# plurigrid/moose

Measured on AMD Instinct MI355X. Metric: replicated fixed(14,23) matmul elems/sec, higher is better.
Workload: dtype fixed(14,23) over Z_2^128 (exact multi-modular int8-MFMA GEMM)

## Files before the change

csrc/gemm_crt.hip:

```cpp
#include <hip/hip_runtime.h>

#include <algorithm>
#include <cmath>
#include <cstdint>
#include <cstdlib>
#include <cstring>
#include <mutex>

#include "hip_attr.h"
#include "moosex.h"
#include "prf_dev.h"
#include "rss_fused.h"

void mx_ws_note(int dev, int64_t want, bool ok);
bool mx_ws_malloc(void** p, int64_t bytes);
void mx_ws_shared_note(void);

namespace {

using u64 = uint64_t;
using u128 = unsigned __int128;
typedef int v4i __attribute__((ext_vector_type(4)));
typedef int v16i __attribute__((ext_vector_type(16)));

// ... 262 lines not shown
    const int r = (int)((g >> 2) & (ROWS - 1));
    const int64_t q = g / (ROWS * 4);
    const int64_t kb = q % nkb, t = q / nkb;
    const int64_t row = t * ROWS + r;
    const int64_t k0 = kb * BK + c * 16;
    uint32_t v[16][NW];
#pragma unroll
    for (int j = 0; j < 16; ++j) {
      const int64_t k = k0 + j;
      T e = 0;
      if (row < R) {
        if (!TRANS) {
          if (k < K) e = mode == 2 ? (T)(x0[row * K + k] + x1[row * K + k]) : x0[row * K + k];
          else if (mode == 1 && k < 2 * K) e = x1[row * K + (k - K)];
        } else {
          if (k < K)
            e = (mode & 1) ? (T)(x0[k * R + row] + x1[k * R + row]) : x0[k * R + row];
          else if (mode == 1 && k < 2 * K) e = x0[(k - K) * R + row];
          else if (mode == 2 && k < 2 * K) e = x1[(k - K) * R + row];
        }
      }
#pragma unroll
      for (int w = 0; w < NW; ++w) v[j][w] = (uint32_t)(e >> (32 * w));
    }
    const int64_t boff = (t * nkb_s + kb) * (int64_t)(ROWS * BK) + img_off(r, c);
    auto emit = [&](int8_t* base) __attribute__((always_inline)) {
    {
      int rr[16];
#pragma unroll
      for (int j = 0; j < 16; ++j) rr[j] = (int)(v[j][0] * tab.mul0);
      v4i o;
#pragma unroll
      for (int u = 0; u < 4; ++u) o[u] = (int)pack4(rr[4 * u], rr[4 * u + 1], rr[4 * u + 2], rr[4 * u + 3]);
      *(v4i*)base = o;
    }
    for (int i = 1; i < n; ++i) {
      const uint32_t w[4] = {tab.w[i][0], tab.w[i][1], tab.w[i][2], tab.w[i][3]};
      const uint32_t neg = tab.neg[i];
      const float p = (float)tab.p[i], rcp = tab.rcp[i];
      int rr[16];
      if constexpr (PK) {
#pragma unroll
        for (int j = 0; j < 16; j += 2)
          residue2<NW>(v[j], v[j + 1], w, neg, p, rcp, rr[j], rr[j + 1]);
      } else {
#pragma unroll
        for (int j = 0; j < 16; ++j) rr[j] = residue<NW>(v[j], w, neg, p, rcp);
      }
      v4i o;
#pragma unroll
      for (int u = 0; u < 4; ++u) o[u] = (int)pack4(rr[4 * u], rr[4 * u + 1], rr[4 * u + 2], rr[4 * u + 3]);
      *(v4i*)(base + i * plane) = o;
    }
    };
    emit(ob + boff);
    if (src.n > 0 && src.dual[b]) {
#pragma unroll
      for (int j = 0; j < 16; ++j) {
        const int64_t k = k0 + j;
        if (row < R && k < K) {
          T e = 0;
#pragma unroll
          for (int w = 0; w < NW; ++w) e |= (T)v[j][w] << (32 * w);
          e += TRANS ? x1[k * R + row] : x1[row * K + k];
#pragma unroll
          for (int w = 0; w < NW; ++w) v[j][w] = (uint32_t)(e >> (32 * w));
        }
      }
      emit(ob + src.dual[b] + boff);
    }
  }
}

struct ShareSrc {
  const void* x = nullptr;
  int kind = 0;
  int frac = 0;
  int j0 = 0;
  uint64_t nonce = 0;
  mxd::KeySrc key;
};
struct SrcPlan {
  const void* x;
  int kind, pad;
  double scale;
  uint64_t nonce;
  int ph[4];
  int64_t off[4];
};

template <bool TRANS, int ROWS, bool PK>
__global__ void __launch_bounds__(256)
    k_crt_prep_src(const SrcPlan s, const mxd::KeySrc keys, int64_t R, int64_t K,
                   int8_t* __restrict__ out, int64_t tiles, int64_t nkb, const PrepTab tab) {
  using T = u128;
  constexpr int NW = 4;
  __shared__ uint32_t rks[1][mxd::kKeyWords];
  __shared__ uint4 xch[4][4][64];
  mxd::stage_keys(rks, keys, 1);
  const int lane = threadIdx.x & 63;
  const int p = lane & 3;
  uint4(*xw)[64] = xch[threadIdx.x >> 6];
  const int n = tab.n;
  const int64_t plane = tiles * nkb * (int64_t)(ROWS * BK);
  const int64_t total = tiles * ROWS * nkb * 4;
  for (int64_t g = blockIdx.x * (int64_t)blockDim.x + threadIdx.x; g < total;
       g += (int64_t)gridDim.x * blockDim.x) {
    const int c = (int)((g >> 2) & 3);
    const int rlow = (int)((g >> 4) & 3);
    const int64_t rest = g >> 6;
    int64_t row, kb, i0, istep;
    if (!TRANS) {
      const int64_t q = rest / (ROWS / 4);
      kb = 4 * (q % (nkb / 4)) + p;
      row = (q / (nkb / 4)) * ROWS + (rest % (ROWS / 4)) * 4 + rlow;
      i0 = row * K + (kb - p) * BK + c * 16;
      istep = 1;
    } else {
      const int64_t q = rest >> 4;
      kb = q % nkb;
      row = (q / nkb) * 256 + 64 * p + (rest & 15) * 4 + rlow;
      i0 = (kb * BK + c * 16) * R + (row - 64 * p);
      istep = R;
    }
    const bool live = row < R;
    const int64_t t = row / ROWS;
    const int r = (int)(row % ROWS);
    uint32_t rr[16][NW], v[16][NW];
#pragma unroll
    for (int jj = 0; jj < 4; ++jj) {
      uint32_t w[16];
      mx::chacha_block(rks[0], s.nonce, mx::ks_block_of((uint64_t)(i0 + (4 * jj + p) * istep)), w);
#pragma unroll
      for (int q = 0; q < 4; ++q)
        xw[q][lane ^ q] = make_uint4(w[4 * q], w[4 * q + 1], w[4 * q + 2], w[4 * q + 3]);
      __builtin_amdgcn_fence(__ATOMIC_RELEASE, "wavefront");
      __builtin_amdgcn_wave_barrier();
      __builtin_amdgcn_fence(__ATOMIC_ACQUIRE, "wavefront");
#pragma unroll
      for (int u = 0; u < 4; ++u) {
        const uint4 e = xw[p][((lane & ~3) | u) ^ p];
        rr[4 * jj + u][0] = live ? e.x : 0u;
        rr[4 * jj + u][1] = live ? e.y : 0u;
        rr[4 * jj + u][2] = live ? e.z : 0u;
        rr[4 * jj + u][3] = live ? e.w : 0u;
      }
      __builtin_amdgcn_fence(__ATOMIC_RELEASE, "wavefront");
      __builtin_amdgcn_wave_barrier();
      __builtin_amdgcn_fence(__ATOMIC_ACQUIRE, "wavefront");
    }
    float kf[16];
    T xp[16];
    if (s.kind == MX_SHARE_F64) {
      double d[16];
#pragma unroll
      for (int j = 0; j < 16; ++j)
        d[j] = live ? ((const double*)s.x)[i0 + 64 * p + j * istep] : 0.0;
#pragma unroll
      for (int j = 0; j < 16; ++j) xp[j] = mxf::share_plain<T>(MX_SHARE_F64, d, j, s.scale);
    } else {
#pragma unroll
      for (int j = 0; j < 16; ++j)
        xp[j] = live ? mxf::share_plain<T>(s.kind, s.x, i0 + 64 * p + j * istep, s.scale) : (T)0;
    }
#pragma unroll
    for (int j = 0; j < 16; ++j) {
      T h = 0;
#pragma unroll
      for (int w = 0; w < NW; ++w) h |= (T)rr[j][w] << (32 * w);
      const T x = xp[j];
      const T other = mxf::share_masked<T>(s.kind, x, h);
#pragma unroll
      for (int w = 0; w < NW; ++w) v[j][w] = (uint32_t)(other >> (32 * w));
      kf[j] = (float)crt_sum_kappa(rr[j][NW - 1], v[j][NW - 1],
                                   (uint32_t)((T)(h + other) >> (32 * (NW - 1))));
    }
    const int64_t boff = (t * nkb + kb) * (int64_t)(ROWS * BK) + img_off(r, c);
    bool has[4];
#pragma unroll
    for (int ph = 0; ph < 4; ++ph)
      has[ph] = s.ph[0] == ph || s.ph[1] == ph || s.ph[2] == ph || s.ph[3] == ph;
    const bool do_r = has[0] || has[2], do_v = has[1] || has[2];
    auto put = [&](int ph, int64_t ioff, const v4i o) __attribute__((always_inline)) {
#pragma unroll
      for (int e = 0; e < 4; ++e)
        if (s.ph[e] == ph) *(v4i*)(out + s.off[e] + ioff + boff) = o;
    };
    auto pack16 = [](const int (&q)[16]) __attribute__((always_inline)) {
      v4i o;
#pragma unroll
      for (int u = 0; u < 4; ++u) o[u] = (int)pack4(q[4 * u], q[4 * u + 1], q[4 * u + 2], q[4 * u + 3]);
      return o;
    };
    const v4i zero = {0, 0, 0, 0};
    {
      int q[16];
#pragma unroll
      for (int j = 0; j < 16; ++j) q[j] = (int)(rr[j][0] * tab.mul0);
      put(0, 0, pack16(q));
#pragma unroll
      for (int j = 0; j < 16; ++j) q[j] = (int)(v[j][0] * tab.mul0);
      put(1, 0, pack16(q));
#pragma unroll
      for (int j = 0; j < 16; ++j) q[j] = (int)((rr[j][0] + v[j][0]) * tab.mul0);
      put(2, 0, pack16(q));
      put(3, 0, zero);
    }
    for (int i = 1; i < n; ++i) {
      const uint32_t w[4] = {tab.w[i][0], tab.w[i][1], tab.w[i][2], tab.w[i][3]};
      const uint32_t neg = tab.neg[i];
      const float pf = (float)tab.p[i], rcp = tab.rcp[i];
      const int64_t ioff = i * plane;
      const float nf = (float)neg;
      auto res4 = [&](const uint32_t (&x)[16][NW], int u, float (&f)[4])
                      __attribute__((always_inline)) {
        if constexpr (PK) {
#pragma unroll
          for (int j = 0; j < 4; j += 2) {
            const f2 g = residue2_f<NW>(x[4 * u + j], x[4 * u + j + 1], w, neg, pf, rcp);
            f[j] = g.x;
            f[j + 1] = g.y;
          }
        } else {
#pragma unroll
          for (int j = 0; j < 4; ++j) f[j] = residue_f<NW>(x[4 * u + j], w, neg, pf, rcp);
        }
      };
      v4i o_r, o_v, o_s;
#pragma unroll
      for (int u = 0; u < 4; ++u) {
        float fr[4], fv[4], fs[4];
        if (do_r) {
          res4(rr, u, fr);
          o_r[u] = (int)pack4((int)fr[0], (int)fr[1], (int)fr[2], (int)fr[3]);
        }
        if (do_v) {
          res4(v, u, fv);
          o_v[u] = (int)pack4((int)fv[0], (int)fv[1], (int)fv[2], (int)fv[3]);
        }
        if (has[2]) {
          if constexpr (PK) {
#pragma unroll
            for (int j = 0; j < 4; j += 2) {
              const f2 g = crt_combine2((f2){fr[j], fr[j + 1]}, (f2){fv[j], fv[j + 1]},
                                        (f2){kf[4 * u + j], kf[4 * u + j + 1]}, nf, pf, rcp);
              fs[j] = g.x;
              fs[j + 1] = g.y;
            }
          } else {
#pragma unroll
            for (int j = 0; j < 4; ++j)
              fs[j] = crt_combine_f(fr[j], fv[j], kf[4 * u + j], nf, pf, rcp);
          }
          o_s[u] = (int)pack4((int)fs[0], (int)fs[1], (int)fs[2], (int)fs[3]);
        }
      }
      put(0, ioff, o_r);
      put(1, ioff, o_v);
      put(2, ioff, o_s);
      put(3, ioff, zero);
    }
  }
}

template <class T>
__global__ void __launch_bounds__(256)
    k_add_pair(const T* __restrict__ a, const T* __restrict__ b, T* __restrict__ o, int64_t n) {
  for (int64_t i = blockIdx.x * (int64_t)blockDim.x + threadIdx.x; i < n;
       i += (int64_t)gridDim.x * blockDim.x)
    o[i] = a[i] + b[i];
}

__device__ inline int64_t xcd_remap(int64_t bid, int64_t nwg) {
  const int64_t q = nwg / 8, r = nwg % 8;
  const int64_t x = bid % 8;
  return (x < r ? x * (q + 1) : r * (q + 1) + (x - r) * q) + bid / 8;
}

constexpr int waitcnt_vm_lgkm0(int vm) { return (vm & 15) | ((vm >> 4) << 14) | (7 << 4); }

__device__ __forceinline__ int centered_mod(int acc, float pf, float rcp, int t16) {
  const int hi = acc >> 16, lo = acc & 0xffff;
  const int s = __mul24(hi, t16) + lo;
  const float fs = (float)s;
  const float qt = __builtin_rintf(fs * rcp);
  return (int)__builtin_fmaf(-qt, pf, fs);
}

template <int WR, int WC, int BN, int MINW>
// ... 158 lines not shown
      qs[e] = 0.f;
#pragma unroll
      for (int k = 0; k < NK; ++k) acc[e][k] = 0;
    }
    const int8_t* src = CR + b * n * ntiles * (int64_t)kCrTile + off;
    for (int i = 0; i < n; ++i) {
      const uint2 v = *(const uint2*)(src + i * ntiles * (int64_t)kCrTile);
      const float rcp = rc.rcp[i];
      int wk[NK];
#pragma unroll
      for (int k = 0; k < NK; ++k) wk[k] = rc.W[i][k];
#pragma unroll
      for (int e = 0; e < 8; ++e) {
        const int c = (int)(int8_t)(((e < 4 ? v.x : v.y) >> (8 * (e & 3))) & 0xff);
        qs[e] = __builtin_fmaf((float)c, rcp, qs[e]);
#pragma unroll
        for (int k = 0; k < NK; ++k) acc[e][k] += __mul24(c, wk[k]);
      }
    }
    const int64_t tm = tile / tiles_n, tn = tile % tiles_n;
    const int bi = blk / NBJ, bj = blk % NBJ;
    const int64_t gcol = tn * BN + bj * 32 + (lane & 31);
    T mw = 0;
#pragma unroll
    for (int k = 0; k < NK; ++k) mw |= (T)rc.Mw[k] << (16 * k);
#pragma unroll
    for (int e = 0; e < 8; ++e) {
      const int ee = hf * 8 + e;
      const int row = (ee & 3) + 8 * (ee >> 2) + 4 * (lane >> 5);
      const int64_t grow = tm * BM + bi * 32 + row;
      T z = 0;
#pragma unroll
      for (int k = 0; k < NK; ++k) z += (T)(int64_t)acc[e][k] << (16 * k);
      const int q = (int)__builtin_rintf(qs[e]);
      z -= (T)(int64_t)q * mw;
      if (grow < M && gcol < N) {
        T* pc = C + (b * M + grow) * N + gcol;
        *pc = accumulate ? (T)(*pc + z) : z;
      }
    }
  }
}

template <int WR, int WC, int BN, int MINW, int STG = kStages, int IL = 0>
__global__ void __launch_bounds__(64 * WR * WC, MINW)
    k_crt_gemm16(const int8_t* __restrict__ RA, const int8_t* __restrict__ RB,
                 int8_t* __restrict__ CR, int tiles_m, int tiles_n, int nkb_all, int gM,
                 const EpiTab ep, int dma_mask, int bcast, int a_nkb, int roll, int amap,
                 int bmap) {
  constexpr int NW = WR * WC;
  constexpr int MI = BM / WR / 16, NJ = BN / WC / 16;
  constexpr int NM = MI * NJ;
  constexpr int kImgB = BN * BK;
  constexpr int kStageBytes = kImg + kImgB;
  constexpr int NPIECE = kStageBytes / 1024;
  constexpr int PPW = NPIECE / NW;
  static_assert(PPW * NW == NPIECE, "stage pieces must split evenly over the waves");
  extern __shared__ __attribute__((aligned(16))) int8_t smem[];
  const int ntiles = tiles_m * tiles_n;
  const int tid_flat = (int)xcd_remap(blockIdx.x, ntiles);
  const int group = tid_flat / (gM * tiles_n);
  const int first_m = group * gM;
  const int gm = tiles_m - first_m < gM ? tiles_m - first_m : gM;
  const int in_group = tid_flat % (gM * tiles_n);
  const int tm = first_m + in_group % gm, tn = in_group / gm;
  const int g = amap < 0 ? (int)((blockIdx.y + ep.n) % gridDim.y) : (int)blockIdx.y;
  const int mi = g % ep.n;
  int nkb = nkb_all;
  const int8_t* ga = RA + ((int64_t)((bcast & 1) ? mi : g) * tiles_m + tm) * a_nkb * (int64_t)kImg;
  const int8_t* gb = RB + ((int64_t)((bcast & 2) ? mi : g) * tiles_n + tn) * nkb_all * (int64_t)kImgB;
  const int8_t* ga2 = ga;
  const int8_t* gb2 = gb;
  int khalf = 1 << 30;
  if (roll) {
    const int nbt = (int)gridDim.y / ep.n;
    const int b2 = (g / ep.n + roll) % nbt;
    ga2 = RA + ((int64_t)(b2 * ep.n + mi) * tiles_m + tm) * a_nkb * (int64_t)kImg -
          (int64_t)a_nkb * kImg;
    khalf = a_nkb;
  } else if (amap < 0) {
    const int sh = 8 * (g / ep.n);
    const int e1 = (amap >> sh) & 7, e2 = (amap >> (sh + 3)) & 7;
    const int f1 = (bmap >> sh) & 7, f2 = (bmap >> (sh + 3)) & 7;
    ga = RA + ((int64_t)(e1 * ep.n + mi) * tiles_m + tm) * a_nkb * (int64_t)kImg;
    ga2 = RA + ((int64_t)(e2 * ep.n + mi) * tiles_m + tm) * a_nkb * (int64_t)kImg -
          (int64_t)a_nkb * kImg;
    gb = RB + ((int64_t)(f1 * ep.n + mi) * tiles_n + tn) * a_nkb * (int64_t)kImgB;
    gb2 = RB + ((int64_t)(f2 * ep.n + mi) * tiles_n + tn) * a_nkb * (int64_t)kImgB -
          (int64_t)a_nkb * kImgB;
    khalf = a_nkb;
    if ((amap >> (sh + 6)) & 1) nkb = a_nkb;
  }

  const int lane = threadIdx.x & 63;
  const int wave = __builtin_amdgcn_readfirstlane(threadIdx.x >> 6);
  const int wr = wave / WC, wc = wave % WC;
  const int co = 16 * ((lane >> 4) ^ swz((lane & 15) >> 2));
  const int rowa = (wr * (BM / WR) + (lane & 15)) * BK + co;
  const int rowb = kImg + (wc * (BN / WC) + (lane & 15)) * BK + co;

  const int8_t* srcs[PPW];
  const int8_t* srcs2[PPW];
  int dsts[PPW], steps[PPW];
#pragma unroll
  for (int t = 0; t < PPW; ++t) {
    const int pc = wave + NW * t;
    const bool is_b = pc >= 16;
    const int pp = is_b ? pc - 16 : pc;
    srcs[t] = (is_b ? gb : ga) + pp * 1024 + lane * 16;
    srcs2[t] = (is_b ? gb2 : ga2) + pp * 1024 + lane * 16;
    dsts[t] = (is_b ? kImg : 0) + pp * 1024;
    steps[t] = is_b ? kImgB : kImg;
  }
  bool dma_on[PPW];
#pragma unroll
  for (int t = 0; t < PPW; ++t) dma_on[t] = (dma_mask >> ((wave + NW * t) >= 16 ? 1 : 0)) & 1;
  auto dma = [&](int kb, int t, int8_t* dst_stage) {
    if (!dma_on[t]) return;
    const int8_t* src = kb >= khalf ? srcs2[t] : srcs[t];
    __builtin_amdgcn_global_load_lds((const void*)(src + (int64_t)kb * steps[t]),
                                     (__attribute__((address_space(3))) void*)(dst_stage + dsts[t]),
                                     16, 0, 0);
  };

  v4i acc[MI][NJ];
#pragma unroll
  for (int i = 0; i < MI; ++i)
#pragma unroll
    for (int j = 0; j < NJ; ++j) acc[i][j] = v4i{0, 0, 0, 0};

  v4i fa0[MI], fb0[NJ], fa1[MI], fb1[NJ];
  const bool no_frags = (dma_mask & 8) != 0;
  auto frags = [&](const int8_t* st, v4i(&fa)[MI], v4i(&fb)[NJ]) {
    if (no_frags) return;
#pragma unroll
    for (int i = 0; i < MI; ++i) fa[i] = *(const v4i*)(st + rowa + i * 16 * BK);
#pragma unroll
    for (int j = 0; j < NJ; ++j) fb[j] = *(const v4i*)(st + rowb + j * 16 * BK);
  };

  constexpr int PRO = IL == 3 ? 4 : STG;
#pragma unroll
  for (int s = 0; s < PRO; ++s)
#pragma unroll
    for (int t = 0; t < PPW; ++t) dma(s < nkb ? s : nkb - 1, t, smem + s * kStageBytes);
  __builtin_amdgcn_s_waitcnt(waitcnt_vm_lgkm0((PRO - 1) * PPW));
  __builtin_amdgcn_s_barrier();
  __builtin_amdgcn_sched_barrier(0);
  frags(smem, fa0, fb0);

  auto step = [&](int kb, int8_t* cur, int8_t* nxt, v4i(&fa)[MI], v4i(&fb)[NJ], v4i(&na)[MI],
                  v4i(&nbf)[NJ]) __attribute__((always_inline)) {
    const int kn = kb + STG < nkb ? kb + STG : nkb - 1;
#pragma unroll MI
    for (int i = 0; i < MI; ++i) {
      if (i == MI / 2) {
        __builtin_amdgcn_s_waitcnt(waitcnt_vm_lgkm0((STG - 2) * PPW));
        __builtin_amdgcn_s_barrier();
        __builtin_amdgcn_sched_barrier(0);
        frags(nxt, na, nbf);
        __builtin_amdgcn_sched_barrier(0);
      }
#pragma unroll NJ
      for (int j = 0; j < NJ; ++j) {
        acc[i][j] = __builtin_amdgcn_mfma_i32_16x16x64_i8(fa[i], fb[j], acc[i][j], 0, 0, 0);
        __builtin_amdgcn_sched_barrier(0);
        const int h = (i - MI / 2) * NJ + j;
#pragma unroll PPW
        for (int t = 0; t < PPW; ++t)
          if (h == (t + 1) * (NM / 2) / PPW - 1) {
            dma(kn, t, cur);
            __builtin_amdgcn_sched_barrier(0);
// ... 284 lines not shown
    return e && e[0] == '0' ? 0 : 1;
  }();
  return v;
}

struct CPlan {
  int n, bn;
  int64_t tiles_m, tiles_n, nkb, a_nkb, ra_bytes, rb_bytes, cr_bytes;
};

CPlan make_cplan(int words, int64_t batch, int64_t M, int64_t N, int64_t K, int mode,
                 bool roll = false) {
  CPlan p;
  p.bn = (crt_kernel() == 3 || crt_kernel() == 5) ? 128 : 256;
  const int64_t kprime = mode ? 2 * K : K;
  p.n = moduli_needed(words, kprime);
  p.tiles_m = (M + BM - 1) / BM;
  p.tiles_n = (N + p.bn - 1) / p.bn;
  p.nkb = round_up(kprime, BK) / BK;
  p.a_nkb = roll ? p.nkb / 2 : p.nkb;
  p.ra_bytes = batch * p.n * p.tiles_m * p.a_nkb * (int64_t)kImg;
  p.rb_bytes = batch * p.n * p.tiles_n * p.nkb * (int64_t)(p.bn * BK);
  p.cr_bytes = batch * p.n * p.tiles_m * p.tiles_n * (int64_t)(BM * p.bn);
  return p;
}

int gemm_group_m() {
  const char* e = std::getenv("MOOSEX_CRT_GROUPM");
  const int v = e ? std::atoi(e) : 8;
  return v >= 1 && v <= 64 ? v : 8;
}

bool prep_packed() {
  static const bool v = [] {
    const char* e = std::getenv("MOOSEX_CRT_PACKED");
    return !(e && e[0] == '0');
  }();
  return v;
}

template <class T>
void launch_prep(const CPlan& p, const Tables& tb, bool is_b, int64_t batch, int64_t R,
                 int64_t K, int64_t xs, const T* X0, const T* X1, int mode, int8_t* out,
                 hipStream_t st, int64_t nkb = -1, int64_t nkb_s = -1,
                 const PrepSrcs& src = PrepSrcs()) {
  if (nkb < 0) nkb = p.nkb;
  if (nkb_s < nkb) nkb_s = nkb;
  const int64_t tiles = is_b ? p.tiles_n : p.tiles_m;
  const int rows = is_b ? p.bn : BM;
  const int64_t work = tiles * nkb * (rows * 4);
  const dim3 grid((unsigned)std::min<int64_t>((work + 255) / 256, 16384), (unsigned)batch);
  static const bool packed_b = [] {
    const char* e = std::getenv("MOOSEX_CRT_PACKED_B");
    return e && e[0] == '1';
  }();
  if (!prep_packed() || (is_b && !packed_b)) {
    if (!is_b)
      hipLaunchKernelGGL((k_crt_prep<T, false, BM, false>), grid, dim3(256), 0, st, X0, X1, R, K,
                         xs, mode, out, tiles, nkb, nkb_s, tb.pa, src);
    else if (rows == 256)
      hipLaunchKernelGGL((k_crt_prep<T, true, 256, false>), grid, dim3(256), 0, st, X0, X1, R, K,
                         xs, mode, out, tiles, nkb, nkb_s, tb.pb, src);
    else
      hipLaunchKernelGGL((k_crt_prep<T, true, 128, false>), grid, dim3(256), 0, st, X0, X1, R, K,
                         xs, mode, out, tiles, nkb, nkb_s, tb.pb, src);
    return;
  }
  if (!is_b)
    hipLaunchKernelGGL((k_crt_prep<T, false, BM>), grid, dim3(256), 0, st, X0, X1, R, K, xs, mode,
                       out, tiles, nkb, nkb_s, tb.pa, src);
  else if (rows == 256)
    hipLaunchKernelGGL((k_crt_prep<T, true, 256>), grid, dim3(256), 0, st, X0, X1, R, K, xs, mode,
                       out, tiles, nkb, nkb_s, tb.pb, src);
  else
    hipLaunchKernelGGL((k_crt_prep<T, true, 128>), grid, dim3(256), 0, st, X0, X1, R, K, xs, mode,
                       out, tiles, nkb, nkb_s, tb.pb, src);
}

bool share_src_ok(const ShareSrc& s) {
  const int kind = s.kind & ~MX_SHARE_MIRROR;
  return s.x && (kind == MX_CROSS_ARITH || kind == MX_SHARE_F64) && s.j0 >= 0 && s.j0 < 3;
}

void launch_prep_src(const CPlan& p, const Tables& tb, bool is_b, const ShareSrc& src, int64_t R,
                     int64_t K, int8_t* out, int64_t entry, hipStream_t st) {
  static const int kSlotsA[4][2] = {{0, 1}, {2, -1}, {1, -1}, {0, -1}};
  static const int kSlotsB[4][2] = {{0, 1}, {1, 2}, {2, -1}, {0, -1}};
  const int kind = src.kind & ~MX_SHARE_MIRROR;
  int jr, jv;
  mxf::share_place(src.j0, (src.kind & MX_SHARE_MIRROR) != 0, &jr, &jv);
  SrcPlan s;
  s.x = src.x;
  s.kind = kind;
  s.pad = 0;
  s.scale = kind == MX_SHARE_F64 ? std::ldexp(1.0, src.frac) : 0.0;
  s.nonce = src.nonce;
  for (int e = 0; e < 4; ++e) {
    const int* sl = is_b ? kSlotsB[e] : kSlotsA[e];
    const bool has_r = sl[0] == jr || sl[1] == jr, has_v = sl[0] == jv || sl[1] == jv;
    s.ph[e] = has_r && has_v ? 2 : has_r ? 0 : has_v ? 1 : 3;
    s.off[e] = e * entry;
  }
  const int64_t tiles = is_b ? p.tiles_n : p.tiles_m;
  const int rows = is_b ? p.bn : BM;
  const int64_t work = tiles * rows * p.a_nkb * 4;
  const dim3 grid((unsigned)std::min<int64_t>(work / 256, 16384));
  if (!is_b)
    hipLaunchKernelGGL((k_crt_prep_src<false, BM, true>), grid, dim3(256), 0, st, s, src.key, R, K,
                       out, tiles, p.a_nkb, tb.pa);
  else if (rows == 256)
    hipLaunchKernelGGL((k_crt_prep_src<true, 256, false>), grid, dim3(256), 0, st, s, src.key, R,
                       K, out, tiles, p.a_nkb, tb.pb);
  else
    hipLaunchKernelGGL((k_crt_prep_src<true, 128, false>), grid, dim3(256), 0, st, s, src.key, R,
                       K, out, tiles, p.a_nkb, tb.pb);
}

int dma_mask() {
  const char* e = std::getenv("MOOSEX_CRT_DMA_MASK");
  return e ? std::atoi(e) : 3;
}

template <int WR, int WC, int BN, int MINW, bool M16, int STG = kStages, int IL = 0>
void launch_variant(const CPlan& p, const Tables& tb, int64_t batch, const int8_t* ra,
                    const int8_t* rb, int8_t* cr, int bcast, int roll, hipStream_t st,
                    int amap = 0, int bmap = 0) {
  constexpr int lds = STG * (kImg + BN * BK);
  const void* fn = M16 ? (const void*)k_crt_gemm16<WR, WC, BN, MINW, STG, IL>
                       : (const void*)k_crt_gemm<WR, WC, BN, MINW>;
  ensure_lds_attr(fn, lds, st);
  const dim3 grid((unsigned)(p.tiles_m * p.tiles_n), (unsigned)(batch * p.n));
  if constexpr (M16)
    hipLaunchKernelGGL((k_crt_gemm16<WR, WC, BN, MINW, STG, IL>), grid, dim3(64 * WR * WC), lds, st, ra,
                       rb, cr, (int)p.tiles_m, (int)p.tiles_n, (int)p.nkb, gemm_group_m(), tb.ep,
                       dma_mask(), bcast, (int)p.a_nkb, roll, amap, bmap);
  else
    hipLaunchKernelGGL((k_crt_gemm<WR, WC, BN, MINW>), grid, dim3(64 * WR * WC), lds, st, ra, rb,
                       cr, (int)p.tiles_m, (int)p.tiles_n, (int)p.nkb, gemm_group_m(), tb.ep,
                       dma_mask(), bcast);
}

void launch_crt_gemm(const CPlan& p, const Tables& tb, int64_t batch, const int8_t* ra,
                     const int8_t* rb, int8_t* cr, int bcast, int roll, hipStream_t st,
                     int amap = 0, int bmap = 0) {
  switch (crt_kernel()) {
    case 1: launch_variant<2, 2, 256, 1, false>(p, tb, batch, ra, rb, cr, bcast, 0, st); break;
    case 2: launch_variant<2, 4, 256, 2, false>(p, tb, batch, ra, rb, cr, bcast, 0, st); break;
    case 4: launch_variant<2, 2, 256, 1, true>(p, tb, batch, ra, rb, cr, bcast, roll, st, amap, bmap); break;
    case 3: launch_variant<2, 2, 128, 2, false>(p, tb, batch, ra, rb, cr, bcast, 0, st); break;
    case 6: launch_variant<2, 4, 256, 2, true>(p, tb, batch, ra, rb, cr, bcast, roll, st, amap, bmap); break;
    case 7: launch_variant<2, 4, 256, 2, true, 4>(p, tb, batch, ra, rb, cr, bcast, roll, st, amap, bmap); break;
    case 8: launch_variant<2, 4, 256, 2, true, 3, 1>(p, tb, batch, ra, rb, cr, bcast, roll, st, amap, bmap); break;
    case 9: launch_variant<2, 4, 256, 2, true, 4, 1>(p, tb, batch, ra, rb, cr, bcast, roll, st, amap, bmap); break;
    case 10: launch_variant<2, 4, 256, 2, true, 3, 2>(p, tb, batch, ra, rb, cr, bcast, roll, st, amap, bmap); break;
    case 11: launch_variant<2, 4, 256, 2, true, 4, 2>(p, tb, batch, ra, rb, cr, bcast, roll, st, amap, bmap); break;
    case 12: launch_variant<2, 2, 256, 1, true, 3, 1>(p, tb, batch, ra, rb, cr, bcast, roll, st, amap, bmap); break;
    case 13: launch_variant<2, 2, 256, 1, true, 4, 1>(p, tb, batch, ra, rb, cr, bcast, roll, st, amap, bmap); break;
    case 14: launch_variant<2, 2, 256, 1, true, 3, 2>(p, tb, batch, ra, rb, cr, bcast, roll, st, amap, bmap); break;
    case 15: launch_variant<2, 2, 256, 1, true, 4, 2>(p, tb, batch, ra, rb, cr, bcast, roll, st, amap, bmap); break;
    case 16: launch_variant<2, 4, 256, 2, true, 5, 3>(p, tb, batch, ra, rb, cr, bcast, roll, st, amap, bmap); break;
    default: launch_variant<2, 2, 128, 2, true>(p, tb, batch, ra, rb, cr, bcast, roll, st, amap, bmap); break;
  }
}

template <class T>
void launch_recon(const CPlan& p, const Tables& tb, int64_t batch, int64_t M, int64_t N,
                  const int8_t* cr, T* C, int accumulate, hipStream_t st) {
  const int64_t work = p.tiles_m * p.tiles_n * (BM * p.bn / 8);
  const int gx = (int)std::min<int64_t>((work + 255) / 256, 16384);
  if (crt_mfma16() && recon_dot4()) {
    const int gx16 = (int)std::min<int64_t>((2 * work + 255) / 256, 16384);
    if (p.bn == 256)
      hipLaunchKernelGGL((k_crt_recon16d<T, 256>), dim3(gx16, (unsigned)batch), dim3(256), 0, st,
                         cr, C, M, N, p.tiles_m, p.tiles_n, accumulate, tb.r4, p.n, tb.rc);
    else
      hipLaunchKernelGGL((k_crt_recon16d<T, 128>), dim3(gx16, (unsigned)batch), dim3(256), 0, st,
                         cr, C, M, N, p.tiles_m, p.tiles_n, accumulate, tb.r4, p.n, tb.rc);
  } else if (crt_mfma16()) {
    const int gx16 = (int)std::min<int64_t>((2 * work + 255) / 256, 16384);
    if (p.bn == 256)
      hipLaunchKernelGGL((k_crt_recon16<T, 256>), dim3(gx16, (unsigned)batch), dim3(256), 0, st,
                         cr, C, M, N, p.tiles_m, p.tiles_n, accumulate, tb.rc);
    else
      hipLaunchKernelGGL((k_crt_recon16<T, 128>), dim3(gx16, (unsigned)batch), dim3(256), 0, st,
// ... 44 lines not shown
    if (!ok) return nullptr;
    w.ptr = q;
    w.bytes = want;
  }
  return w.ptr;
}

template <class T>
int run_crt(int64_t batch, int64_t M, int64_t N, int64_t K, const T* A0, const T* A1,
            int64_t a_bstride, const T* B0, const T* B1, int64_t b_bstride,
            const int8_t* rb_pre, int mode, T* C, int accumulate, hipStream_t st,
            int64_t roll = 0) {
  constexpr int words = sizeof(T) / 8;
  if (roll && (mode != 1 || K % BK || !crt_mfma16() || a_bstride == 0 || batch < 2 ||
               roll % batch == 0))
    return -7;
  const CPlan p = make_cplan(words, batch, M, N, K, mode, roll != 0);
  if (p.n < 0) return -6;
  if ((mode ? 2 * K : K) > (1 << 15)) return -6;
  const Tables& tb = tables_for(words, p.n);
  const int64_t need = p.ra_bytes + (rb_pre ? 0 : p.rb_bytes) + p.cr_bytes;
  int8_t* ws = (int8_t*)workspace(need, st);
  if (!ws) return -4;
  int8_t* ra = ws;
  int8_t* cr = ra + p.ra_bytes;
  const int8_t* rb = rb_pre;
  const bool a_bc = batch > 1 && a_bstride == 0;
  const bool b_bc = batch > 1 && b_bstride == 0 && !rb_pre;
  if (!rb) {
    int8_t* rbw = cr + p.cr_bytes;
    launch_prep<T>(p, tb, true, b_bc ? 1 : batch, N, K, b_bstride, B0, B1, mode, rbw, st);
    rb = rbw;
  }
  if (roll)
    launch_prep<T>(p, tb, false, batch, M, K, a_bstride, A0, A0, 0, ra, st, p.a_nkb);
  else
    launch_prep<T>(p, tb, false, a_bc ? 1 : batch, M, K, a_bstride, A0, A1, mode, ra, st);
  launch_crt_gemm(p, tb, batch, ra, rb, cr, (a_bc ? 1 : 0) | (b_bc ? 2 : 0),
                  (int)(((roll % batch) + batch) % batch), st);
  launch_recon<T>(p, tb, batch, M, N, cr, C, accumulate, st);
  const hipError_t e = hipGetLastError();
  return e != hipSuccess ? -100 - (int)e : 0;
}

template <class T>
int run_crt_asym(int64_t M, int64_t N, int64_t K, const T* S0, const T* S1, const T* T0,
                 const T* T1, int rolled, T* C, hipStream_t st, const ShareSrc* xs = nullptr,
                 const ShareSrc* ys = nullptr) {
  constexpr int words = sizeof(T) / 8;
  if (K % BK || !crt_mfma16()) return -7;
  if (2 * K > (1 << 15)) return -6;
  const CPlan p = make_cplan(words, 3, M, N, K, 1, true);
  if (p.n < 0) return -6;
  const Tables& tb = tables_for(words, p.n);
  const int64_t sa = M * K, sb = K * N;
  const T* a[3];
  const T* b[3];
  const T* c[3];
  const T* d[3];
  for (int q = 0; q < 3; ++q) {
    a[q] = S0 + q * sa;
    b[q] = rolled ? S0 + ((q + 1) % 3) * sa : S1 + q * sa;
    c[q] = T0 + q * sb;
    d[q] = rolled ? T0 + ((q + 1) % 3) * sb : T1 + q * sb;
  }
  int na, nb, amap, bmap;
  const int64_t a_entry = p.n * p.tiles_m * p.a_nkb * (int64_t)kImg;
  const int64_t b_entry = p.n * p.tiles_n * p.a_nkb * (int64_t)(p.bn * BK);
  auto pmap = [](int e0, int e1, int e2, int e3, int e4) {
    return (int)(0x80000000u | (unsigned)e0 | (1u << 6) | ((unsigned)(e1 | (e2 << 3)) << 8) |
                 ((unsigned)(e3 | (e4 << 3)) << 16));
  };
  if (rolled) {
    na = 4;
    nb = 4;
    amap = pmap(0, 1, 2, 1, 3);
    bmap = pmap(0, 1, 2, 3, 2);
  } else {
    na = 5;
    nb = 5;
    amap = pmap(0, 1, 2, 3, 4);
    bmap = pmap(0, 1, 2, 3, 4);
  }
  const int64_t ra_bytes = na * a_entry, rb_bytes = nb * b_entry;
  static const bool asum = [] {
    const char* e = std::getenv("MOOSEX_CRT_ASUM");
    return !(e && e[0] == '0');
  }();
  static const bool dual = [] {
    const char* e = std::getenv("MOOSEX_CRT_DUAL");
    return !(e && e[0] == '0');
  }();
  const bool duals = rolled && dual;
  if (xs || ys) {
    if (words != 2 || !duals) return -7;
    if (xs && (K % 256 || !share_src_ok(*xs))) return -7;
    if (ys && (N % 256 || !share_src_ok(*ys))) return -7;
  }
  const int64_t sum_bytes = asum && !duals ? round_up(sa * (int64_t)sizeof(T), 256) : 0;
  int8_t* ws = (int8_t*)workspace(ra_bytes + rb_bytes + p.cr_bytes + sum_bytes, st);
  if (!ws) return -4;
  int8_t* ra = ws;
  int8_t* cr = ra + ra_bytes;
  int8_t* rb = cr + p.cr_bytes;
  T* a01 = sum_bytes ? (T*)(rb + rb_bytes) : nullptr;
  if (a01)
    hipLaunchKernelGGL((k_add_pair<T>), dim3((unsigned)std::min<int64_t>((sa + 255) / 256, 65536)),
                       dim3(256), 0, st, a[0], b[0], a01, sa);
  const int64_t kn = p.a_nkb;
  PrepSrcs sa_, sb_;
  auto put = [](PrepSrcs& q, const T* x0, const T* x1, int mode, int64_t dual = 0) {
    q.x0[q.n] = x0;
    q.x1[q.n] = x1;
    q.mode[q.n] = mode;
    q.dual[q.n] = dual;
    ++q.n;
  };
  if (duals) {
    put(sa_, a[2], a[2], 0);
    put(sa_, a[1], a[1], 0);
    put(sa_, a[0], b[0], 0, -3 * a_entry);
    put(sb_, d[1], c[1], 0, -b_entry);
    put(sb_, d[2], d[0], 0, -3 * b_entry);
    if (ys)
      launch_prep_src(p, tb, true, *ys, N, K, rb, b_entry, st);
    else
      launch_prep<T>(p, tb, true, sb_.n, N, K, 0, nullptr, nullptr, 0, rb + 2 * b_entry, st, kn,
                     kn, sb_);
    if (xs)
      launch_prep_src(p, tb, false, *xs, M, K, ra, a_entry, st);
    else
      launch_prep<T>(p, tb, false, sa_.n, M, K, 0, nullptr, nullptr, 0, ra + a_entry, st, kn, kn,
                     sa_);
  } else {
    if (a01)
      put(sa_, a01, a01, 0);
    else
      put(sa_, a[0], b[0], 2);
    put(sb_, c[0], d[0], 3);
    put(sb_, c[1], d[1], 3);
    if (rolled) {
      for (const T* e : {a[2], a[1], a[0]}) put(sa_, e, e, 0);
      for (const T* f : {d[1], d[2]}) put(sb_, f, f, 0);
    } else {
      for (const T* e : {b[1], a[1], a[2], b[2]}) put(sa_, e, e, 0);
      for (const T* f : {d[1], d[2], c[2]}) put(sb_, f, f, 0);
    }
    launch_prep<T>(p, tb, true, sb_.n, N, K, 0, nullptr, nullptr, 0, rb, st, kn, kn, sb_);
    launch_prep<T>(p, tb, false, sa_.n, M, K, 0, nullptr, nullptr, 0, ra, st, kn, kn, sa_);
  }
  launch_crt_gemm(p, tb, 3, ra, rb, cr, 0, 0, st, amap, bmap);
  launch_recon<T>(p, tb, 3, M, N, cr, C, 0, st);
  const hipError_t e = hipGetLastError();
  return e != hipSuccess ? -100 - (int)e : 0;
}

}

extern "C" {

int mx_gemm_asym(int words, int64_t M, int64_t N, int64_t K, const void* S0, const void* S1,
                 const void* T0, const void* T1, int rolled, void* C, void* stream) {
  if (M == 0 || N == 0) return 0;
  if (!rolled && (!S1 || !T1)) return -2;
  hipStream_t st = (hipStream_t)stream;
  if (words == 1)
    return run_crt_asym<u64>(M, N, K, (const u64*)S0, (const u64*)S1, (const u64*)T0,
                             (const u64*)T1, rolled, (u64*)C, st);
  if (words == 2)
    return run_crt_asym<u128>(M, N, K, (const u128*)S0, (const u128*)S1, (const u128*)T0,
                              (const u128*)T1, rolled, (u128*)C, st);
  return -2;
}

int mx_gemm_asym_src(int words, int64_t M, int64_t N, int64_t K, const void* S0, const void* T0,
                     const int64_t* xsrc, const int64_t* ysrc, void* C, void* stream) {
  if (M == 0 || N == 0) return 0;
  if (words != 2) return -7;
  if ((!xsrc && !S0) || (!ysrc && !T0)) return -2;
  ShareSrc sx, sy;
  auto fill = [](ShareSrc& s, const int64_t* a) {
    s.x = (const void*)(intptr_t)a[0];
    s.kind = (int)a[1];
    s.frac = (int)a[2];
    s.j0 = (int)a[3];
    const uint32_t* slot[1] = {(const uint32_t*)(intptr_t)a[4]};
    s.key = mxd::keysrc_slots(slot, 1);
    s.nonce = (uint64_t)a[5];
  };
  if (xsrc) fill(sx, xsrc);
  if (ysrc) fill(sy, ysrc);
  if ((xsrc && !sx.key.slot[0]) || (ysrc && !sy.key.slot[0])) return -2;
  return run_crt_asym<u128>(M, N, K, (const u128*)S0, nullptr, (const u128*)T0, nullptr, 1,
                            (u128*)C, (hipStream_t)stream, xsrc ? &sx : nullptr,
                            ysrc ? &sy : nullptr);
}

int mx_crt_moduli(int words, int64_t kprime) {
  if (words != 1 && words != 2) return -2;
  return moduli_needed(words, kprime);
}

int mx_crt_tables(int words, int n, int32_t* p_out, uint8_t* wa_out, uint8_t* wb_out,
                  int32_t* nega_out, int32_t* negb_out, uint16_t* W_out, uint16_t* Mw_out) {
  if ((words != 1 && words != 2) || n < 1 || n > kMaxMod) return -2;
  const Tables& t = tables_for(words, n);
  for (int i = 0; i < n; ++i) {
    p_out[i] = t.ep.p[i];
    for (int j = 0; j < 16; ++j) {
      wa_out[i * 16 + j] = (uint8_t)(t.pa.w[i][j / 4] >> (8 * (j % 4)));
      wb_out[i * 16 + j] = (uint8_t)(t.pb.w[i][j / 4] >> (8 * (j % 4)));
    }
    nega_out[i] = (int32_t)t.pa.neg[i];
// ... 124 lines not shown
```

Baseline: 1.511 billion.

## Replace all-zero residue planes with a single shared zero strip

When a share source has a phase that produces an all-zero residue image, that image is no longer materialised in the workspace. Each operand instead gets one small zero strip ahead of its buffer, and the GEMM pointer maps are remapped so those entries point at the strip. This is meant to cut prep-kernel writes and workspace size for the share-source path. The cost is extra pointer-selection logic in the GEMM kernel and a more complex remapping of the amap/bmap encoding.

Result: faster. 1.542 billion, median of 6 (+2.0%).

```diff
diff --git a/csrc/gemm_crt.hip b/csrc/gemm_crt.hip
--- a/csrc/gemm_crt.hip
+++ b/csrc/gemm_crt.hip
@@ -368,12 +368,14 @@
 };
 struct SrcPlan {
   const void* x;
-  int kind, pad;
+  int kind, strip;
   double scale;
   uint64_t nonce;
   int ph[4];
   int64_t off[4];
+  int64_t zoff;
 };
+constexpr int kZeroStrip = 7;
 
 template <bool TRANS, int ROWS, bool PK>
 __global__ void __launch_bounds__(256)
@@ -491,6 +493,7 @@
       for (int j = 0; j < 16; ++j) q[j] = (int)((rr[j][0] + v[j][0]) * tab.mul0);
       put(2, 0, pack16(q));
       put(3, 0, zero);
+      if (s.strip && t == 0) *(v4i*)(out + s.zoff + boff) = zero;
     }
     for (int i = 1; i < n; ++i) {
       const uint32_t w[4] = {tab.w[i][0], tab.w[i][1], tab.w[i][2], tab.w[i][3]};
@@ -815,12 +818,13 @@
     const int sh = 8 * (g / ep.n);
     const int e1 = (amap >> sh) & 7, e2 = (amap >> (sh + 3)) & 7;
     const int f1 = (bmap >> sh) & 7, f2 = (bmap >> (sh + 3)) & 7;
-    ga = RA + ((int64_t)(e1 * ep.n + mi) * tiles_m + tm) * a_nkb * (int64_t)kImg;
-    ga2 = RA + ((int64_t)(e2 * ep.n + mi) * tiles_m + tm) * a_nkb * (int64_t)kImg -
-          (int64_t)a_nkb * kImg;
-    gb = RB + ((int64_t)(f1 * ep.n + mi) * tiles_n + tn) * a_nkb * (int64_t)kImgB;
-    gb2 = RB + ((int64_t)(f2 * ep.n + mi) * tiles_n + tn) * a_nkb * (int64_t)kImgB -
-          (int64_t)a_nkb * kImgB;
+    const int64_t sa_ = (int64_t)a_nkb * kImg, sb_ = (int64_t)a_nkb * kImgB;
+    ga = e1 == kZeroStrip ? RA - sa_ : RA + ((int64_t)(e1 * ep.n + mi) * tiles_m + tm) * sa_;
+    ga2 = (e2 == kZeroStrip ? RA - sa_ : RA + ((int64_t)(e2 * ep.n + mi) * tiles_m + tm) * sa_) -
+          sa_;
+    gb = f1 == kZeroStrip ? RB - sb_ : RB + ((int64_t)(f1 * ep.n + mi) * tiles_n + tn) * sb_;
+    gb2 = (f2 == kZeroStrip ? RB - sb_ : RB + ((int64_t)(f2 * ep.n + mi) * tiles_n + tn) * sb_) -
+          sb_;
     khalf = a_nkb;
     if ((amap >> (sh + 6)) & 1) nkb = a_nkb;
   }
@@ -1271,24 +1275,34 @@
   return s.x && (kind == MX_CROSS_ARITH || kind == MX_SHARE_F64) && s.j0 >= 0 && s.j0 < 3;
 }
 
-void launch_prep_src(const CPlan& p, const Tables& tb, bool is_b, const ShareSrc& src, int64_t R,
-                     int64_t K, int8_t* out, int64_t entry, hipStream_t st) {
+void src_phases(bool is_b, const ShareSrc& src, int (&ph)[4]) {
   static const int kSlotsA[4][2] = {{0, 1}, {2, -1}, {1, -1}, {0, -1}};
   static const int kSlotsB[4][2] = {{0, 1}, {1, 2}, {2, -1}, {0, -1}};
-  const int kind = src.kind & ~MX_SHARE_MIRROR;
   int jr, jv;
   mxf::share_place(src.j0, (src.kind & MX_SHARE_MIRROR) != 0, &jr, &jv);
+  for (int e = 0; e < 4; ++e) {
+    const int* sl = is_b ? kSlotsB[e] : kSlotsA[e];
+    const bool has_r = sl[0] == jr || sl[1] == jr, has_v = sl[0] == jv || sl[1] == jv;
+    ph[e] = has_r && has_v ? 2 : has_r ? 0 : has_v ? 1 : 3;
+  }
+}
+
+void launch_prep_src(const CPlan& p, const Tables& tb, bool is_b, const ShareSrc& src, int64_t R,
+                     int64_t K, int8_t* out, int64_t entry, const int (&ph)[4],
+                     const int (&at)[4], int64_t zoff, hipStream_t st) {
+  const int kind = src.kind & ~MX_SHARE_MIRROR;
   SrcPlan s;
   s.x = src.x;
   s.kind = kind;
-  s.pad = 0;
+  s.strip = 0;
   s.scale = kind == MX_SHARE_F64 ? std::ldexp(1.0, src.frac) : 0.0;
   s.nonce = src.nonce;
+  s.zoff = zoff;
   for (int e = 0; e < 4; ++e) {
-    const int* sl = is_b ? kSlotsB[e] : kSlotsA[e];
-    const bool has_r = sl[0] == jr || sl[1] == jr, has_v = sl[0] == jv || sl[1] == jv;
-    s.ph[e] = has_r && has_v ? 2 : has_r ? 0 : has_v ? 1 : 3;
-    s.off[e] = e * entry;
+    const bool z = at[e] == kZeroStrip;
+    s.ph[e] = z ? -1 : ph[e];
+    s.off[e] = z ? 0 : at[e] * entry;
+    s.strip |= z;
   }
   const int64_t tiles = is_b ? p.tiles_n : p.tiles_m;
   const int rows = is_b ? p.bn : BM;
@@ -1499,7 +1513,6 @@
     amap = pmap(0, 1, 2, 3, 4);
     bmap = pmap(0, 1, 2, 3, 4);
   }
-  const int64_t ra_bytes = na * a_entry, rb_bytes = nb * b_entry;
   static const bool asum = [] {
     const char* e = std::getenv("MOOSEX_CRT_ASUM");
     return !(e && e[0] == '0');
@@ -1514,12 +1527,32 @@
     if (xs && (K % 256 || !share_src_ok(*xs))) return -7;
     if (ys && (N % 256 || !share_src_ok(*ys))) return -7;
   }
+  static const bool zstrip = [] {
+    const char* e = std::getenv("MOOSEX_ZERO_STRIP");
+    return !(e && e[0] == '0');
+  }();
+  int aph[4], bph[4], aat[4] = {0, 1, 2, 3}, bat[4] = {0, 1, 2, 3};
+  int64_t a_strip = 0, b_strip = 0;
+  auto plan_src = [&](bool is_b, const ShareSrc& s, int (&ph)[4], int (&at)[4], int& n, int& map,
+                      int64_t& strip) {
+    src_phases(is_b, s, ph);
+    int m = 0;
+    for (int e = 0; e < 4; ++e) at[e] = zstrip && ph[e] == 3 ? kZeroStrip : m++;
+    if (m == n) return;
+    n = m;
+    strip = p.a_nkb * (int64_t)(is_b ? p.bn * BK : kImg);
+    for (int sh : {0, 8, 11, 16, 19}) map = (map & ~(7 << sh)) | (at[(map >> sh) & 7] << sh);
+  };
+  if (xs) plan_src(false, *xs, aph, aat, na, amap, a_strip);
+  if (ys) plan_src(true, *ys, bph, bat, nb, bmap, b_strip);
+  const int64_t ra_bytes = na * a_entry, rb_bytes = nb * b_entry;
   const int64_t sum_bytes = asum && !duals ? round_up(sa * (int64_t)sizeof(T), 256) : 0;
-  int8_t* ws = (int8_t*)workspace(ra_bytes + rb_bytes + p.cr_bytes + sum_bytes, st);
+  int8_t* ws = (int8_t*)workspace(
+      a_strip + ra_bytes + p.cr_bytes + b_strip + rb_bytes + sum_bytes, st);
   if (!ws) return -4;
-  int8_t* ra = ws;
+  int8_t* ra = ws + a_strip;
   int8_t* cr = ra + ra_bytes;
-  int8_t* rb = cr + p.cr_bytes;
+  int8_t* rb = cr + p.cr_bytes + b_strip;
   T* a01 = sum_bytes ? (T*)(rb + rb_bytes) : nullptr;
   if (a01)
     hipLaunchKernelGGL((k_add_pair<T>), dim3((unsigned)std::min<int64_t>((sa + 255) / 256, 65536)),
@@ -1540,12 +1573,12 @@
     put(sb_, d[1], c[1], 0, -b_entry);
     put(sb_, d[2], d[0], 0, -3 * b_entry);
     if (ys)
-      launch_prep_src(p, tb, true, *ys, N, K, rb, b_entry, st);
+      launch_prep_src(p, tb, true, *ys, N, K, rb, b_entry, bph, bat, -b_strip, st);
     else
       launch_prep<T>(p, tb, true, sb_.n, N, K, 0, nullptr, nullptr, 0, rb + 2 * b_entry, st, kn,
                      kn, sb_);
     if (xs)
-      launch_prep_src(p, tb, false, *xs, M, K, ra, a_entry, st);
+      launch_prep_src(p, tb, false, *xs, M, K, ra, a_entry, aph, aat, -a_strip, st);
     else
       launch_prep<T>(p, tb, false, sa_.n, M, K, 0, nullptr, nullptr, 0, ra + a_entry, st, kn, kn,
                      sa_);
```
